# jessicabonnie/dandd

Hardware: AMD Instinct MI355X
Metric: Gbp/s sketched over k-sweep (higher is better)
Workload: dtype u64; 1 GPU; cfg2: 10 x 50 Mbp synthetic FASTA on this GPU (10 over 1 GPU(s)) resident in HBM, HLL log2m=14, k-sweep 4-40 (K=37), leaf sketches + root union + all cardinalities + delta; genomes_per_gpu=10, bases_per_genome=50000000, kmin=4, kmax=40, log2m=14, parallelism=genomes sharded over 1 GPU(s)

## Files before the change

dandd_amd/csrc/dd_api.hip:

```cpp
#include "dd_ctx.h"

thread_local std::string g_err;

extern "C" {

int dd_abi_version(void) { return DD_ABI_VERSION; }

const char* dd_last_error(void) { return g_err.c_str(); }

dd_ctx* dd_create(int device, int log2m, int canonical) {
    if (log2m < 4 || log2m > 20) {
        fail(DD_EINVAL, "log2m=%d outside 4..20", log2m);
        return nullptr;
    }
    int ndev = 0;
    hipError_t e = hipGetDeviceCount(&ndev);
    if (e != hipSuccess || ndev <= 0) {
        fail(DD_ENODEV, "no HIP device visible (%s): libdandd_hip has no CPU path",
             e == hipSuccess ? "device count 0" : hipGetErrorString(e));
        return nullptr;
    }
    if (device < 0 || device >= ndev) {
        fail(DD_ENODEV, "device %d not in 0..%d", device, ndev - 1);
        return nullptr;
// ... 6 lines not shown
    if (strncmp(prop.gcnArchName, "gfx950", 6) != 0) {
        fail(DD_ENODEV, "device %d is %s; this library is built for gfx950 only", device,
             prop.gcnArchName);
        return nullptr;
    }
    dd_ctx* c = new dd_ctx();
    c->device = device;
    c->p = log2m;
    c->canonical = canonical ? 1 : 0;
    c->bucket_budget = std::min<size_t>((size_t)48 << 30, std::max<size_t>((size_t)16 << 30, prop.totalGlobalMem / 6));
    DeviceGuard g(device);
    if (hipEventCreateWithFlags(&c->stage[0].free, hipEventDisableTiming) != hipSuccess ||
        hipEventCreateWithFlags(&c->stage[1].free, hipEventDisableTiming) != hipSuccess) {
        fail(DD_ENODEV, "hipEventCreate failed");
        delete c;
        return nullptr;
    }
    return c;
}

void dd_destroy(dd_ctx* c) {
    if (!c) return;
    DeviceGuard g(c->device);
    (void)hipStreamSynchronize(c->stream);
    (void)dd_comm_destroy(c);
    for (auto& v : c->spans)
        for (auto& s : v) {
            (void)hipEventDestroy(s.a);
            (void)hipEventDestroy(s.b);
        }
    for (auto e : c->pool) (void)hipEventDestroy(e);
    for (auto& pe : c->plans) pe.jobtab.release();
    for (DevBuf* b : {&c->tokens, &c->scratch, &c->tables, &c->fasta, &c->regs, &c->ptrs, &c->hist,
                      &c->est, &c->ord, &c->bitmaps, &c->bigmaps, &c->exact, &c->buckets, &c->gram, &c->synth, &c->masks, &c->emit, &c->hits, &c->pat[0], &c->pat[1]})
        b->release();
    for (StageSet& s : c->stage) {
        if (s.free) (void)hipEventDestroy(s.free);
        for (HostBuf* b : {&s.tables, &s.jobs, &s.rows}) b->release();
    }
    c->ingest.release();
    for (int i = 0; i < 8; ++i)
        if (c->side[i]) {
            (void)hipStreamDestroy(c->side[i]);
            (void)hipEventDestroy(c->side_done[i]);
        }
    if (c->side_go) (void)hipEventDestroy(c->side_go);
    delete c;
}

int dd_set_stream(dd_ctx* c, void* hip_stream) {
    if (check_ctx(c)) return DD_EINVAL;
    hipStream_t next = static_cast<hipStream_t>(hip_stream);
    if (next != c->stream) {
        DeviceGuard g(c->device);
        DD_HIP(hipDeviceSynchronize());
        c->stream = next;
    }
    return DD_OK;
}

int dd_synchronize(dd_ctx* c) {
    if (check_ctx(c)) return DD_EINVAL;
    DeviceGuard g(c->device);
    DD_HIP(hipStreamSynchronize(c->stream));
    return DD_OK;
}

// ... 109 lines not shown
```

dandd_amd/csrc/dd_ctx.h:

```cpp
#pragma once
#include "../../include/dandd_hip.h"
#include <sched.h>
#include <stdarg.h>
#include <stdio.h>
#include <stdlib.h>
#include <string.h>
#include <algorithm>
#include <string>
#include <thread>
#include <vector>
#include "dd_common.h"
#include "dd_io.h"
#include "dd_kernels.h"
#include "dd_plan.h"

extern thread_local std::string g_err;
inline int fail(int code, const char* fmt, ...) {
    char buf[512];
    va_list ap;
    va_start(ap, fmt), vsnprintf(buf, sizeof buf, fmt, ap), va_end(ap);
    g_err = buf;
    return code;
}
#define DD_HIP(expr)                                                                                                     \
// ... 42 lines not shown
    std::vector<dd::FileBuf*> file_pool;
    hipStream_t copy_stream_b = nullptr;
    hipStream_t copy_stream = nullptr, out_stream = nullptr;
    PipeSet pipe[2];
    bool no_gpu_inflate = false;
    int inflate_refusals = 0;
    bool inflate_retry = false;
    bool inflate_retry_counts = false;
    struct TextSink { uint8_t* const* out; const size_t* caps; size_t* lens; bool short_buffer; };
    TextSink* text_sink = nullptr;
    int calls = 0;
    double ms[4] = {0, 0, 0, 0};
    void release() {
        for (dd::FileBuf*& fb : file_pool) delete fb, fb = nullptr;
        for (PipeSet& s : pipe) s.release();
        for (hipStream_t* s : {&copy_stream, &copy_stream_b, &out_stream})
            if (*s) (void)hipStreamDestroy(*s), *s = nullptr;
    }
};

struct StageSet { HostBuf tables, jobs, rows; hipEvent_t free = nullptr; };

struct dd_ctx {
    int device = 0, p = 14, canonical = 1;
    hipStream_t stream = nullptr;
    bool timing = false;
    std::vector<TimedSpan> spans[DD_KERNEL_COUNT];
    std::vector<hipEvent_t> pool;
    DevBuf tokens, scratch, tables, fasta, regs, ptrs, hist, est, ord, bitmaps, bigmaps, exact, buckets, gram, synth;
    DevBuf masks;
    DevBuf emit;
    DevBuf hits;
    DevBuf pat[2];
    StageSet stage[2];
    int stage_cur = 0;
    struct PlanEntry {
        bool valid = false;
        int kmin = 0, kmax = 0;
        std::vector<size_t> sizes;
        dd::PlanKnobs knobs;
        std::vector<dd::SweepClass> classes;
        std::vector<size_t> job_off;
        DevBuf jobtab;
        unsigned long long last_use = 0;
    };
    PlanEntry plans[8];
    unsigned long long plan_clock = 0;
    IngestState ingest;
    hipStream_t side[8] = {};
    hipEvent_t side_done[8] = {}, side_go = nullptr;
    size_t bucket_budget = (size_t)16 << 30;
    uint64_t st_tokens = 0, st_updates = 0;
    int st_blocks = 0;
    int k2_path = 0;
    void* comm = nullptr;
    int comm_rank = 0, comm_world = 1;
    unsigned long long comm_calls[2] = {0, 0};
};
struct DeviceGuard {
    int prev = -1;
    explicit DeviceGuard(int dev) {
        (void)hipGetDevice(&prev);
        if (prev != dev) (void)hipSetDevice(dev);
        else prev = -1;
    }
    ~DeviceGuard() { if (prev >= 0) (void)hipSetDevice(prev); }
// ... 149 lines not shown
```

dandd_amd/csrc/dd_kernels.h:

```cpp
#pragma once
#include <atomic>
#include <type_traits>
#include <vector>
#include <hip/hip_runtime.h>
#include <stddef.h>
#include <stdint.h>

namespace dd {

template <typename F>
void dispatch_bool(bool b, const F& f) {
    if (b) f(std::true_type{});
    else f(std::false_type{});
}
template <auto Kern, int STATIC_LDS = 0, typename... Args>
void launch_full_lds(dim3 grid, dim3 block, size_t lds_bytes, hipStream_t st, Args... args) {
    static std::atomic<unsigned long long> allowed{0};
    int dev = 0;
    (void)hipGetDevice(&dev);
    const unsigned long long bit = 1ull << (dev & 63);
    if (!(allowed.load(std::memory_order_relaxed) & bit)) {
        if (hipFuncSetAttribute(reinterpret_cast<const void*>(Kern), hipFuncAttributeMaxDynamicSharedMemorySize, 160 * 1024 - STATIC_LDS) != hipSuccess)
            (void)hipGetLastError();
        allowed.fetch_or(bit, std::memory_order_relaxed);
// ... 3 lines not shown

struct TokenStream {
    uint32_t* codes;
    uint32_t* bad;
    unsigned long long* ntok;
};

constexpr int kPackThreads = 256;
constexpr int kPackBytesPerThread = 64;
constexpr int kPackChunk = kPackThreads * kPackBytesPerThread;
constexpr int kSegTokens = 64;

inline size_t pack_chunks(size_t n) { return (n + kPackChunk - 1) / kPackChunk; }
inline size_t pack_scratch_bytes(size_t n) { return ((pack_chunks(n) + 1) * 4 + 2) * sizeof(long long); }
inline size_t codes_words(size_t n) { return ((n + 63) / 64 + 1) * 4; }
inline size_t bad_words(size_t n) { return ((n + 63) / 64 + 1) * 2; }

struct PackGenome {
    const uint8_t* fa;
    size_t n;
    size_t nchunks;
    long long* scratch;
    TokenStream out;
};
void launch_pack_batch(const PackGenome* tab_dev, int ngenomes, size_t max_chunks, hipStream_t st);

struct SweepGenome {
    const uint32_t* codes;
    const uint32_t* bad;
    const unsigned long long* ntok;
    uint8_t* regs;
    uint32_t* bitmap;
    uint32_t* bigmap;
};

constexpr int kBitmapMaxK = 9;
constexpr int kBitmapWords = 10924;
constexpr int kBitmapStride = 11008;
inline constexpr int bitmap_offset(int k) {
    int off = 0;
    for (int j = 1; j < k; ++j) off += (j < 3) ? 1 : (1 << (2 * j - 5));
    return off;
}
inline constexpr int bitmap_words(int k) { return (k < 3) ? 1 : (1 << (2 * k - 5)); }
constexpr int kBigmapMinK = 10, kBigmapMaxK = 11;
constexpr int kBigmapSliceWords = 1 << 15;
inline constexpr int bigmap_last_k(int log2m) { return log2m >= 20 ? 11 : (log2m >= 19 ? 10 : 0); }
inline constexpr int bigmap_bits(int k, bool canon) { return (canon && (k & 1)) ? 2 * k - 1 : 2 * k; }
inline constexpr int bigmap_slices(int k, bool canon) { return 1 << (bigmap_bits(k, canon) - 20); }
inline constexpr size_t bigmap_offset_words(int k, bool canon) {
    size_t off = 0;
    for (int j = kBigmapMinK; j < k; ++j) off += (size_t)bigmap_slices(j, canon) * kBigmapSliceWords;
    return off;
}
struct SweepJob {
    int genome;
    int kfirst;
    int nk;
    int krow;
    unsigned tile_begin, tile_end;
    int slice;
};
constexpr int kBucketMode = 5;
constexpr int kBucketFromLog2m = 17;
constexpr unsigned kRaiseQueueRecords = 128;
constexpr unsigned kRaiseQueueBytes = 16 * kRaiseQueueRecords * 4;
struct SweepPlan {
    int log2m;
    int canonical;
    int threads;
    int lds_bytes;
    int queue_off = 0;
    int mode;
    int logg = 0;
    int nb_log2 = 0;
    unsigned cap_chunks = 0;
    int nepochs = 0;
};
void launch_sweep(const SweepGenome* genomes_dev, const SweepJob* jobs_dev, int njobs, int kclass,
                  const SweepPlan& plan, hipStream_t st);

struct BucketRow {
    uint8_t* regs;
    uint32_t* area;
    uint32_t* cursor;
    uint32_t* fill;
    uint16_t* seg;
    uint8_t* filter;
    uint32_t* ones;
};
struct ScatterParams {
    const BucketRow* rows;
    int K;
    int logg;
    unsigned cap_chunks;
    int nb_log2;
};
void launch_scatter(const SweepGenome* genomes_dev, const SweepJob* jobs_dev, int njobs, int kclass,
                    const SweepPlan& plan, const ScatterParams& sp, hipStream_t st, bool first_epoch);
void launch_replay(const BucketRow* rows_dev, int ngenomes, int K, int k0, int nks, const SweepPlan& plan, hipStream_t st, bool first_epoch);
int sweep_max_lds_bytes();
void launch_bitmap(const SweepGenome* genomes_dev, const SweepJob* jobs_dev, int njobs, int kfirst, int klast,
                   int canonical, hipStream_t st);
void launch_bigmap(const SweepGenome* genomes_dev, const SweepJob* jobs_dev, int njobs, int canonical, hipStream_t st);
void launch_bigmap_finish(const SweepGenome* genomes_dev, int ngenomes, int kfirst, int klast, int kmin, int log2m,
                          int canonical, hipStream_t st);
void launch_bitmap_finish(const SweepGenome* genomes_dev, int ngenomes, int kfirst, int klast, int kmin,
                          int log2m, hipStream_t st);

void launch_union(const uint8_t* const* in_dev, int n, size_t len, uint8_t* out_dev, hipStream_t st);
void launch_hist(const uint8_t* regs_dev, int njobs, int log2m, uint32_t* hist_dev, hipStream_t st);
void launch_progressive(const uint8_t* leaf_dev, int n, int K, int log2m, const int32_t* ord_dev,
                        int norder, uint32_t* hist_dev, hipStream_t st);
// ... 201 lines not shown
```

dandd_amd/csrc/dd_plan.h:

```cpp
#pragma once
#include <stddef.h>

#include <vector>

#include "dd_kernels.h"

namespace dd {

constexpr int kBitmapClass = -1;
constexpr int kBigmapClass = -2;

struct SweepClass {
    int kclass;
    int kfirst, klast;
    SweepPlan plan;
    std::vector<SweepJob> jobs;
    std::vector<size_t> epoch_begin;
};

struct PlanKnobs {
    size_t bucket_e0_tiles = 0;
    size_t bucket_emax_tiles = 0;
    size_t bucket_cap_chunks = 0;
    size_t bucket_budget = (size_t)16 << 30;
    bool bigmap_any_size = false;
    static PlanKnobs from_env();
    bool operator==(const PlanKnobs& o) const {
        return bucket_e0_tiles == o.bucket_e0_tiles && bucket_emax_tiles == o.bucket_emax_tiles && bucket_cap_chunks == o.bucket_cap_chunks &&
               bucket_budget == o.bucket_budget && bigmap_any_size == o.bigmap_any_size;
    }
};

bool plan_bigmap_range(int log2m, int kmin, int kmax, const PlanKnobs& knobs, const size_t* nbytes, int ngenomes, int* ka, int* kb);
std::vector<SweepClass> plan_sweep(int log2m, int canonical, const size_t* nbytes, int ngenomes, int kmin,
                                   int kmax, const PlanKnobs& knobs);

struct BucketLayout {
    int K = 0, per_genome = 0;
    std::vector<int> slot;
    size_t table = 0, cursors = 0, filters = 0, ones = 0, fills = 0, areas = 0;
    size_t cursor_stride = 256, filter_bytes = 0, ones_bytes = 0, fill_bytes = 0, seg_off = 0, area_bytes = 0;
    size_t zero_begin = 0, zero_bytes = 0, total = 0;
};
BucketLayout bucket_layout(const std::vector<SweepClass>& classes, int log2m, int ngenomes, int kmin, int kmax);
void bucket_rows(const BucketLayout& lay, char* base, uint8_t* regs, int log2m, int ngenomes, BucketRow* rows);

}
```

dandd_amd/csrc/dd_plan.hip:

```cpp
#include "dd_plan.h"

#include <stdlib.h>

#include <algorithm>

namespace dd {

PlanKnobs PlanKnobs::from_env() {
    PlanKnobs k;
    k.bigmap_any_size = getenv("DD_BIGMAP_ANY_SIZE") != nullptr;
    if (const char* e = getenv("DD_BUCKET_E0")) k.bucket_e0_tiles = (size_t)std::max(1, atoi(e));
    if (const char* e = getenv("DD_BUCKET_EMAX")) k.bucket_emax_tiles = (size_t)std::max(1, atoi(e));
    if (const char* e = getenv("DD_BUCKET_CAP")) k.bucket_cap_chunks = (size_t)std::max(1, atoi(e));
    if (const char* e = getenv("DD_BUCKET_GB")) k.bucket_budget = (size_t)std::max(1, atoi(e)) << 30;
    return k;
}

namespace {

constexpr int kThreads = 1024;
constexpr size_t kTileTokens = (size_t)kThreads * kSegTokens;

size_t tiles_of(size_t nbytes) { return (nbytes + kTileTokens - 1) / kTileTokens; }
size_t align_to(size_t v, size_t a) { return (v + a - 1) / a * a; }

SweepJob make_job(int genome, int kfirst, int nk, int kmin, size_t t0, size_t t1) {
    SweepJob j;
    j.genome = genome;
    j.kfirst = kfirst;
    j.nk = nk;
    j.krow = kfirst - kmin;
    j.tile_begin = (unsigned)t0;
    j.tile_end = (unsigned)t1;
    j.slice = 0;
    return j;
}

}

bool plan_bigmap_range(int log2m, int kmin, int kmax, const PlanKnobs& knobs, const size_t* nbytes, int ngenomes, int* ka, int* kb) {
    int last = log2m >= kBucketFromLog2m ? bigmap_last_k(log2m) : 0;
    size_t total = 0;
    for (int g = 0; g < ngenomes; ++g) total += nbytes[g];
    const size_t avg = ngenomes > 0 ? total / (size_t)ngenomes : 0;
    const size_t tiles = (size_t)1 << std::max(0, log2m - 17);
    while (!knobs.bigmap_any_size && last >= kBigmapMinK && avg < tiles * ((size_t)1 << (2 * last))) --last;
    const int a = std::max(kmin, kBigmapMinK), b = std::min(kmax, last);
    if (a > b) return false;
    if (ka) *ka = a;
    if (kb) *kb = b;
    return true;
}

std::vector<SweepClass> plan_sweep(int log2m, int canonical, const size_t* nbytes, int ngenomes, int kmin,
                                   int kmax, const PlanKnobs& knobs) {
    std::vector<SweepClass> classes;
    if (ngenomes <= 0 || kmin < 1 || kmax > 64 || kmin > kmax) return classes;
    const int p = log2m;
    const size_t m = (size_t)1 << p;
    const bool bucket_mode = p >= kBucketFromLog2m;
    const size_t lds_budget = std::max<size_t>(80 * 1024, m);
    const int slots = (int)std::min<size_t>(64, lds_budget / m);
    const bool use_bitmaps = kmin <= kBitmapMaxK;
    int big_ka = 0, big_kb = 0;
    const bool use_big = plan_bigmap_range(p, kmin, kmax, knobs, nbytes, ngenomes, &big_ka, &big_kb);

    const int lo0 = use_big ? big_kb + 1 : (use_bitmaps ? kBitmapMaxK + 1 : 1);
    const struct { int kc, ka, kb; } class_tab[6] = {
        {kBitmapClass, 1, use_bitmaps ? kBitmapMaxK : 0}, {kBigmapClass, big_ka, use_big ? big_kb : 0},
        {0, lo0, 16}, {1, 17, 32}, {3, 33, 48}, {2, 49, 64}};

    size_t total_tiles = 0, max_tiles = 0;
    for (int g = 0; g < ngenomes; ++g) {
        total_tiles += tiles_of(nbytes[g]);
        max_tiles = std::max(max_tiles, tiles_of(nbytes[g]));
    }

    int bucket_logg = std::max(1, p - 17);
    while (bucket_logg > 0 && (m >> bucket_logg) / 2 < 16) --bucket_logg;
    const int nb_log2 = std::max(0, p - 16);
    std::vector<size_t> epoch_edge;
    size_t epoch_longest = 0, bucket_row_tokens = 0;
    if (bucket_mode) {
        int bucketed_ks = 0;
// ... 201 lines not shown
```

dandd_amd/csrc/dd_sketch_api.hip:

```cpp
#include "dd_ctx.h"

static int ensure_side_streams(dd_ctx* c, int n) {
    if (!c->side_go) DD_HIP(hipEventCreateWithFlags(&c->side_go, hipEventDisableTiming));
    for (int i = 0; i < std::min(n, 8); ++i) {
        if (c->side[i]) continue;
        DD_HIP(hipStreamCreateWithFlags(&c->side[i], hipStreamNonBlocking));
        DD_HIP(hipEventCreateWithFlags(&c->side_done[i], hipEventDisableTiming));
    }
    return DD_OK;
}

struct SideLanes {
    dd_ctx* c;
    int lane = 0;
    template <class F>
    int run(bool fork, F&& launch) {
        const int l = lane & 7;
        if (!fork) return launch(c->stream), DD_OK;
        DD_HIP(hipStreamWaitEvent(c->side[l], c->side_go, 0));
        launch(c->side[l]);
        DD_HIP(hipEventRecord(c->side_done[l], c->side[l]));
        DD_HIP(hipStreamWaitEvent(c->stream, c->side_done[l], 0));
        ++lane;
        return DD_OK;
    }
};

struct Bitmaps { uint32_t* small = nullptr; uint32_t* big = nullptr; size_t big_stride = 0; };
static int reserve_bitmaps(dd_ctx* c, const dd::PlanKnobs& knobs, const size_t* nbytes, int ngenomes, int kmin, int kmax, Bitmaps& bm) {
    int rc, ka = 0, kb = 0;
    if (kmin <= dd::kBitmapMaxK) {
        const size_t bbytes = (size_t)ngenomes * dd::kBitmapStride * sizeof(uint32_t);
        if ((rc = c->bitmaps.reserve(bbytes))) return rc;
        bm.small = static_cast<uint32_t*>(c->bitmaps.p);
        DD_HIP(hipMemsetAsync(bm.small, 0, bbytes, c->stream));
    }
    if (dd::plan_bigmap_range(c->p, kmin, kmax, knobs, nbytes, ngenomes, &ka, &kb)) {
        bm.big_stride = dd::bigmap_offset_words(kb + 1, c->canonical != 0);
        const size_t bbytes = (size_t)ngenomes * bm.big_stride * sizeof(uint32_t);
        if ((rc = c->bigmaps.reserve(bbytes))) return rc;
        bm.big = static_cast<uint32_t*>(c->bigmaps.p);
        DD_HIP(hipMemsetAsync(bm.big, 0, bbytes, c->stream));
    }
    return DD_OK;
}

static int cached_plan(dd_ctx* c, StageSet& stage, const dd::PlanKnobs& knobs, const size_t* nbytes, int ngenomes, int kmin, int kmax, dd_ctx::PlanEntry** out) {
    dd_ctx::PlanEntry* pc = &c->plans[0];
    for (auto& pe : c->plans) {
        if (pe.valid && pe.kmin == kmin && pe.kmax == kmax && pe.knobs == knobs && pe.sizes.size() == (size_t)ngenomes &&
            std::equal(pe.sizes.begin(), pe.sizes.end(), nbytes)) {
            pe.last_use = ++c->plan_clock;
            *out = &pe;
            return DD_OK;
        }
        if (pe.last_use < pc->last_use) pc = &pe;
    }
    pc->last_use = ++c->plan_clock;
    pc->valid = false;
    pc->classes = dd::plan_sweep(c->p, c->canonical, nbytes, ngenomes, kmin, kmax, knobs);
    size_t job_bytes = 0;
    pc->job_off.assign(pc->classes.size(), 0);
    for (size_t i = 0; i < pc->classes.size(); ++i) {
        pc->job_off[i] = job_bytes;
        job_bytes += align_up(sizeof(dd::SweepJob) * pc->classes[i].jobs.size(), 256);
    }
    int rc;
    if ((rc = pc->jobtab.reserve(job_bytes))) return rc;
    if ((rc = stage.jobs.reserve(job_bytes))) return rc;
    for (size_t i = 0; i < pc->classes.size(); ++i)
        if ((rc = upload(c, stage.jobs, static_cast<char*>(pc->jobtab.p) + pc->job_off[i], pc->classes[i].jobs.data(),
                         sizeof(dd::SweepJob) * pc->classes[i].jobs.size(), pc->job_off[i])))
            return rc;
    pc->kmin = kmin;
    pc->kmax = kmax;
    pc->knobs = knobs;
    pc->sizes.assign(nbytes, nbytes + ngenomes);
    pc->valid = true;
    *out = pc;
    return DD_OK;
}

static int upload_bucket_rows(dd_ctx* c, StageSet& stage, const std::vector<dd::SweepClass>& classes, int ngenomes, int kmin, int kmax, uint8_t* regs_dev,
                              const dd::BucketRow** rows_dev) {
    const dd::BucketLayout lay = dd::bucket_layout(classes, c->p, ngenomes, kmin, kmax);
    if (!lay.total) return DD_OK;
    std::vector<dd::BucketRow> rtab((size_t)ngenomes * lay.K);
    int rc;
    if ((rc = c->buckets.reserve(lay.total))) return rc;
    if ((rc = stage.rows.reserve(lay.cursors - lay.table))) return rc;
    char* bb = static_cast<char*>(c->buckets.p);
    dd::bucket_rows(lay, bb, regs_dev, c->p, ngenomes, rtab.data());
    DD_HIP(hipMemsetAsync(bb + lay.zero_begin, 0, lay.zero_bytes, c->stream));
    if ((rc = upload(c, stage.rows, bb + lay.table, rtab.data(), sizeof(dd::BucketRow) * rtab.size(), 0))) return rc;
    *rows_dev = reinterpret_cast<const dd::BucketRow*>(bb + lay.table);
    return DD_OK;
}

static void launch_lds_class(dd_ctx* c, const dd::SweepClass& sc, const dd::SweepGenome* gt, const dd::SweepJob* jt, int ngenomes, int kmin, hipStream_t ks) {
    if (sc.kclass == dd::kBitmapClass) {
        dd::launch_bitmap(gt, jt, (int)sc.jobs.size(), sc.kfirst, sc.klast, c->canonical, ks);
        dd::launch_bitmap_finish(gt, ngenomes, sc.kfirst, sc.klast, kmin, c->p, ks);
    } else if (sc.kclass == dd::kBigmapClass) {
        dd::launch_bigmap(gt, jt, (int)sc.jobs.size(), c->canonical, ks);
        dd::launch_bigmap_finish(gt, ngenomes, sc.kfirst, sc.klast, kmin, c->p, c->canonical, ks);
    } else {
        dd::launch_sweep(gt, jt, (int)sc.jobs.size(), sc.kclass, sc.plan, ks);
    }
}

static int launch_classes(dd_ctx* c, const dd_ctx::PlanEntry& plan, const dd::SweepGenome* gtab, const dd::BucketRow* rows, int ngenomes, int kmin, int kmax, int* blocks) {
    const int K = kmax - kmin + 1;
    size_t lds_jobs = 0;
    int lds_classes = 0, nepochs = 0, rc;
    for (const dd::SweepClass& sc : plan.classes) {
        if (sc.plan.mode != dd::kBucketMode) lds_jobs += sc.jobs.size(), ++lds_classes;
        else nepochs = sc.plan.nepochs;
    }
    const bool side = lds_classes > 1 && lds_jobs < 12000, side_b = nepochs > 1;
    if ((side || side_b) && (rc = ensure_side_streams(c, side_b ? (int)plan.classes.size() : lds_classes))) return rc;
    Span phase(c, DD_KERNEL_SWEEP, side || side_b);
    if (side || side_b) DD_HIP(hipEventRecord(c->side_go, c->stream));
    SideLanes lanes{c};
    for (size_t i = 0; i < plan.classes.size(); ++i) {
        const dd::SweepClass& sc = plan.classes[i];
        const dd::SweepJob* jobs = reinterpret_cast<const dd::SweepJob*>(static_cast<char*>(plan.jobtab.p) + plan.job_off[i]);
        const bool bucket = sc.plan.mode == dd::kBucketMode, on_lane = side_b || (side && !bucket);
        rc = lanes.run(on_lane, [&](hipStream_t ks) {
            if (!bucket) {
                Span span(c, DD_KERNEL_SWEEP, !on_lane);
                launch_lds_class(c, sc, gtab, jobs, ngenomes, kmin, ks);
            }
            const dd::ScatterParams sp{rows, K, sc.plan.logg, sc.plan.cap_chunks, sc.plan.nb_log2};
            for (int e = 0; bucket && e < sc.plan.nepochs; ++e) {
                const size_t j0 = sc.epoch_begin[e], j1 = sc.epoch_begin[e + 1];
                if (j1 == j0) continue;
                Span span(c, DD_KERNEL_SWEEP, !on_lane);
                dd::launch_scatter(gtab, jobs + j0, (int)(j1 - j0), sc.kclass, sc.plan, sp, ks, e == 0);
                dd::launch_replay(rows, ngenomes, K, sc.kfirst - kmin, sc.klast - sc.kfirst + 1, sc.plan, ks, e == 0);
            }
        });
        if (rc) return rc;
        *blocks += (int)sc.jobs.size();
    }
    DD_HIP(hipGetLastError());
    return DD_OK;
}

extern "C" {

int dd_sketch_device(dd_ctx* c, const uint8_t* const* fasta_dev, const size_t* nbytes, int ngenomes,
                     int kmin, int kmax, uint8_t* regs_dev) {
    if (check_ctx(c)) return DD_EINVAL;
    if (ngenomes < 0 || !regs_dev || (ngenomes && (!fasta_dev || !nbytes)))
        return fail(DD_EINVAL, "null argument");
    if (kmin < 1 || kmax > 64 || kmin > kmax) return fail(DD_EINVAL, "k range %d..%d outside 1..64", kmin, kmax);
    uint64_t tokens_ub = 0;
    for (int g = 0; g < ngenomes; ++g) {
        if (nbytes[g] && !fasta_dev[g]) return fail(DD_EINVAL, "genome %d: null buffer", g);
        if (reinterpret_cast<uintptr_t>(fasta_dev[g]) & 15)
            return fail(DD_EINVAL, "genome %d: device buffer must be 16-byte aligned", g);
        tokens_ub += nbytes[g];
    }
    DeviceGuard guard(c->device);
    const size_t K = (size_t)(kmax - kmin + 1), m = (size_t)1 << c->p;
    DD_HIP(hipMemsetAsync(regs_dev, 0, (size_t)ngenomes * K * m, c->stream));
    if (!ngenomes) return DD_OK;

    dd::PlanKnobs knobs = dd::PlanKnobs::from_env();
    if (!getenv("DD_BUCKET_GB")) knobs.bucket_budget = c->bucket_budget;
    std::vector<dd::PackGenome> ptab;
    size_t max_chunks = 0;
    Bitmaps bm;
    int rc;
    if ((rc = layout_tokens(c, fasta_dev, nbytes, ngenomes, ptab, max_chunks))) return rc;
    if ((rc = reserve_bitmaps(c, knobs, nbytes, ngenomes, kmin, kmax, bm))) return rc;
    std::vector<dd::SweepGenome> gtab(ngenomes);
    for (int g = 0; g < ngenomes; ++g) {
        const dd::TokenStream& ts = ptab[g].out;
        gtab[g] = dd::SweepGenome{ts.codes, ts.bad, ts.ntok, regs_dev + (size_t)g * K * m,
                                  bm.small ? bm.small + (size_t)g * dd::kBitmapStride : nullptr,
                                  bm.big ? bm.big + (size_t)g * bm.big_stride : nullptr};
    }

    const size_t pack_off = align_up(sizeof(dd::SweepGenome) * ngenomes, 256);
    const size_t gtab_bytes = pack_off + align_up(sizeof(dd::PackGenome) * ngenomes, 256);
    if ((rc = c->tables.reserve(gtab_bytes))) return rc;
    StageSet& stage = c->stage[c->stage_cur ^= 1];
    DD_HIP(hipEventSynchronize(stage.free));
    if ((rc = stage.tables.reserve(gtab_bytes))) return rc;
    char* tdev = static_cast<char*>(c->tables.p);
    if ((rc = upload(c, stage.tables, tdev, gtab.data(), sizeof(dd::SweepGenome) * ngenomes, 0))) return rc;
    if ((rc = upload(c, stage.tables, tdev + pack_off, ptab.data(), sizeof(dd::PackGenome) * ngenomes, pack_off))) return rc;
    {
        Span sp(c, DD_KERNEL_PACK);
        dd::launch_pack_batch(reinterpret_cast<const dd::PackGenome*>(tdev + pack_off), ngenomes, max_chunks, c->stream);
    }
    DD_HIP(hipGetLastError());

    dd_ctx::PlanEntry* plan = nullptr;
    const dd::BucketRow* rows_dev = nullptr;
    int blocks = 0;
    if ((rc = cached_plan(c, stage, knobs, nbytes, ngenomes, kmin, kmax, &plan))) return rc;
    if ((rc = upload_bucket_rows(c, stage, plan->classes, ngenomes, kmin, kmax, regs_dev, &rows_dev))) return rc;
    DD_HIP(hipEventRecord(stage.free, c->stream));
    if ((rc = launch_classes(c, *plan, reinterpret_cast<const dd::SweepGenome*>(tdev), rows_dev, ngenomes, kmin, kmax, &blocks))) return rc;
    c->st_tokens = tokens_ub;
    c->st_updates = tokens_ub * (uint64_t)K;
    c->st_blocks = blocks;
    return DD_OK;
}

int dd_sketch_buffer(dd_ctx* c, const uint8_t* fasta, size_t nbytes, int kmin, int kmax, uint8_t* regs) {
    if (check_ctx(c)) return DD_EINVAL;
    if (!regs || (nbytes && !fasta)) return fail(DD_EINVAL, "null argument");
    if (kmin < 1 || kmax > 64 || kmin > kmax) return fail(DD_EINVAL, "k range %d..%d outside 1..64", kmin, kmax);
    DeviceGuard guard(c->device);
    const size_t K = (size_t)(kmax - kmin + 1), m = (size_t)1 << c->p;
    int rc;
    dd::FileBuf fq;
    if (dd::has_plus_line(fasta, nbytes)) {
        if (!fq.reserve(nbytes + 16)) return fail(DD_ENOMEM, "out of host memory");
        fq.len = nbytes = dd::fastq_to_fasta(fasta, nbytes, fq.p);
        fasta = fq.p;
    }
    if ((rc = c->fasta.reserve(nbytes + 16))) return rc;
    if ((rc = c->regs.reserve(K * m))) return rc;
    if (nbytes) DD_HIP(hipMemcpyAsync(c->fasta.p, fasta, nbytes, hipMemcpyHostToDevice, c->stream));
    const uint8_t* ptrs[1] = {static_cast<const uint8_t*>(c->fasta.p)};
    const size_t ns[1] = {nbytes};
    if ((rc = dd_sketch_device(c, ptrs, ns, 1, kmin, kmax, static_cast<uint8_t*>(c->regs.p)))) return rc;
    DD_HIP(hipMemcpyAsync(regs, c->regs.p, K * m, hipMemcpyDeviceToHost, c->stream));
    DD_HIP(hipStreamSynchronize(c->stream));
    return DD_OK;
}

}
```

dandd_amd/csrc/dd_sweep.hip:

```cpp
#include "dd_common.h"
#include "dd_kernels.h"
#include "dd_k1.h"

namespace dd {
namespace {

template <int KC, bool CANON, bool CHECK, typename Win>
DD_D void sweep_token(const Win& win, int run, int kfirst, int nk, int p, RaiseQueue& s) {
    constexpr bool QUEUE = KC != 0;
    asm volatile("" : "+s"(nk));
    int j = 0;
#pragma unroll 1
    for (; j + 1 < nk; j += 2) {
        const int k = kfirst + j;
        const bool ok0 = !CHECK || run >= k, ok1 = !CHECK || run > k;
        const unsigned long long okm0 = CHECK ? __builtin_amdgcn_ballot_w64(run >= k) : ~0ull, okm1 = CHECK ? __builtin_amdgcn_ballot_w64(run > k) : ~0ull;
        if (CHECK && !okm0) return;
        sweep_update2<QUEUE, CHECK>(s, (uint32_t)j, win.template hash<CANON>(k), okm0, ok0,
                                    (uint32_t)j + 1u, win.template hash<CANON>(k + 1), okm1, ok1, p);
    }
    if (j < nk) {
        const int k = kfirst + j;
        const unsigned long long okm = CHECK ? __builtin_amdgcn_ballot_w64(run >= k) : ~0ull;
        if (!CHECK || okm) sweep_update<QUEUE, CHECK>(s, (uint32_t)j, win.template hash<CANON>(k), okm, !CHECK || run >= k, p);
    }
}

template <int KC, bool CANON>
__global__ __launch_bounds__(1024) void sweep_kernel(const SweepGenome* __restrict__ genomes,
                                                    const SweepJob* __restrict__ jobs, int p, uint32_t queue_off) {
    lds_starts_at_zero();
    const SweepJob job = jobs[blockIdx.x];
    const SweepGenome g = genomes[job.genome];
    const int nk = job.nk, kfirst = job.kfirst;
    const uint32_t m = 1u << p;
    const unsigned long long ntok = gload8u(g.ntok);
    uint8_t* const slab = g.regs + ((size_t)job.krow << p);

    TileIn next;
    fetch_tile(g, job, ntok, job.tile_begin, next);

    {
        uint4* z = reinterpret_cast<uint4*>(g_lds);
        const uint32_t n16 = (uint32_t)nk * (m >> 4);
        for (uint32_t i = threadIdx.x; i < n16; i += blockDim.x) z[i] = load16_fresh(slab + (size_t)i * 16);
    }
    __syncthreads();

    const int kmaxg = kfirst + nk - 1;
    RaiseQueue s;
    s.base = queue_off + (uint32_t)__builtin_amdgcn_readfirstlane(threadIdx.x >> 6) * (kRaiseQueueRecords * 4u);
    s.dense = (KC != 0 && queue_off) ? kRaiseDense : 0u;
    s.waiting = 0;

    for (unsigned tile = job.tile_begin; tile < job.tile_end; ++tile) {
        const TileIn cur = next;
        fetch_tile(g, job, ntok, tile + 1, next);
        if (!__any(cur.live)) continue;
        SweepWindows<KC> win;
        walk_segment(cur, win, [&](auto clean, int run) {
            if constexpr (decltype(clean)::value) {
                sweep_token<KC, CANON, false>(win, 0, kfirst, nk, p, s);
            } else {
                if (__all(run >= kmaxg)) sweep_token<KC, CANON, false>(win, run, kfirst, nk, p, s);
                else sweep_token<KC, CANON, true>(win, run, kfirst, nk, p, s);
            }
        });
    }
    if (s.dense) sweep_drain(s);
    __syncthreads();

    const uint4* l4 = reinterpret_cast<const uint4*>(g_lds);
    uint32_t* gw = reinterpret_cast<uint32_t*>(slab);
    const uint32_t n16 = (uint32_t)nk * (m >> 4);
    for (uint32_t i = threadIdx.x; i < n16; i += blockDim.x) {
        const uint4 lv = l4[i];
        const uint4 gv = load16_fresh(slab + (size_t)i * 16);
        const uint32_t l[4] = {lv.x, lv.y, lv.z, lv.w};
        const uint32_t o[4] = {gv.x, gv.y, gv.z, gv.w};
#pragma unroll
        for (int q = 0; q < 4; ++q) {
            uint32_t old = o[q];
            uint32_t mx = bmax4(old, l[q]);
            while (mx != old) {
                uint32_t prev = gcas32(&gw[4 * i + q], old, mx);
                if (prev == old) break;
                old = prev;
                mx = bmax4(old, l[q]);
            }
        }
    }
}

__constant__ int c_bitmap_off[kBitmapMaxK + 2] = {0, bitmap_offset(1), bitmap_offset(2), bitmap_offset(3),
                                                 bitmap_offset(4), bitmap_offset(5), bitmap_offset(6),
                                                 bitmap_offset(7), bitmap_offset(8), bitmap_offset(9),
                                                 kBitmapWords};
static_assert(kBitmapMaxK == 9 && bitmap_offset(9) + bitmap_words(9) == kBitmapWords &&
              kBitmapWords + kBitmapMaxK < kBitmapStride, "bitmap layout");

template <bool CANON>
__global__ __launch_bounds__(1024) __attribute__((amdgpu_num_sgpr(72))) void bitmap_kernel(const SweepGenome* __restrict__ genomes,
                                                     const SweepJob* __restrict__ jobs) {
    const SweepJob job = jobs[blockIdx.x];
    const SweepGenome g = genomes[job.genome];
    const int kfirst = job.kfirst, klast = job.kfirst + job.nk - 1;
    const unsigned long long ntok = gload8u(g.ntok);
    const int w0 = c_bitmap_off[kfirst], w1 = c_bitmap_off[klast + 1];
    uint32_t* const bits = reinterpret_cast<uint32_t*>(g_lds) - w0;
    uint32_t kmask = __builtin_amdgcn_readfirstlane(((2u << klast) - 1u) & ~((1u << kfirst) - 1u));
    uint32_t* const complete = g.bitmap + kBitmapWords;
    __shared__ uint32_t have[kBitmapMaxK + 2];
    __shared__ uint32_t flagged;
    if (threadIdx.x == 0) {
        uint32_t f = 0;
        for (int k = kfirst; k <= klast; ++k)
            if (load4_fresh(complete + k)) f |= 1u << k;
        flagged = f;
    }
    if (threadIdx.x <= kBitmapMaxK) have[threadIdx.x] = 0;
    __syncthreads();
    kmask = __builtin_amdgcn_readfirstlane(kmask & ~flagged);
// ... 156 lines not shown
#pragma unroll
        for (int w = 0; w < 4; ++w) {
            const uint32_t bw = ((w & 2) ? sb.y : sb.x) >> ((w & 1) * 16);
#pragma unroll 4
            for (int i = 0; i < 16; ++i) {
                const uint32_t c = (cws[w] >> (2 * i)) & 3u;
                run = ((bw >> i) & 1u) ? 0 : run + 1;
                win.push(c);
                record(bigmap_index<CANON>(win.fw, win.rc, k), run >= k);
            }
        }
    }
    __syncthreads();
    for (int i = threadIdx.x; i < kBigmapSliceWords; i += blockDim.x) {
        const uint32_t mine = bits[i];
        if (mine && (mine & ~load4_fresh(home + i))) gor32(home + i, mine);
    }
}

template <bool CANON>
__global__ __launch_bounds__(1024) void bigmap_finish_kernel(const SweepGenome* __restrict__ genomes,
                                                            int kfirst, int kmin, int p, int tile_log2) {
    lds_starts_at_zero();
    const SweepGenome g = genomes[blockIdx.y];
    const int k = kfirst + (int)blockIdx.x;
    const uint32_t b = blockIdx.z;
    const uint32_t* bm = g.bigmap + bigmap_offset_words(k, CANON);
    const uint32_t nw = (uint32_t)bigmap_slices(k, CANON) * kBigmapSliceWords;
    finish_tile(g.regs + ((size_t)(k - kmin) << p) + ((size_t)b << tile_log2), tile_log2, b, p, [&](const auto& emit) {
        for_each_set_bit(bm, nw, [&](uint32_t idx) { emit(bigmap_kmer<CANON>(idx, k)); });
    });
}

}

int sweep_max_lds_bytes() { return 160 * 1024; }

void launch_bitmap(const SweepGenome* genomes, const SweepJob* jobs, int njobs, int kfirst, int klast,
                   int canonical, hipStream_t st) {
    if (njobs <= 0 || kfirst < 1 || klast > kBitmapMaxK || klast < kfirst) return;
    const size_t lds = (size_t)(bitmap_offset(klast) + bitmap_words(klast) - bitmap_offset(kfirst)) * 4;
    dispatch_bool(canonical != 0, [&](auto cn) {
        launch_full_lds<bitmap_kernel<decltype(cn)::value>, 256>(dim3((unsigned)njobs), dim3(1024), lds, st, genomes, jobs);
    });
}

void launch_bitmap_finish(const SweepGenome* genomes, int ngenomes, int kfirst, int klast, int kmin, int log2m,
                          hipStream_t st) {
    if (ngenomes <= 0 || klast < kfirst) return;
    const int tile_log2 = std::min(log2m, 16);
    hipLaunchKernelGGL(bitmap_finish_kernel, dim3((unsigned)(klast - kfirst + 1), (unsigned)ngenomes, 1u << (log2m - tile_log2)), dim3(1024),
                       (size_t)1 << tile_log2, st, genomes, kfirst, kmin, log2m, tile_log2);
}

void launch_bigmap(const SweepGenome* genomes, const SweepJob* jobs, int njobs, int canonical, hipStream_t st) {
    if (njobs <= 0) return;
    dispatch_bool(canonical != 0, [&](auto cn) {
        launch_full_lds<bigmap_kernel<decltype(cn)::value>>(dim3((unsigned)njobs), dim3(1024), (size_t)kBigmapSliceWords * 4, st, genomes, jobs);
    });
}

void launch_bigmap_finish(const SweepGenome* genomes, int ngenomes, int kfirst, int klast, int kmin, int log2m,
                          int canonical, hipStream_t st) {
    if (ngenomes <= 0 || klast < kfirst) return;
    const int tile_log2 = std::min(log2m, 17);
    const dim3 grid((unsigned)(klast - kfirst + 1), (unsigned)ngenomes, 1u << (log2m - tile_log2));
    dispatch_bool(canonical != 0, [&](auto cn) {
        launch_full_lds<bigmap_finish_kernel<decltype(cn)::value>>(grid, dim3(1024), (size_t)1 << tile_log2, st, genomes, kfirst, kmin, log2m, tile_log2);
    });
}

void launch_sweep(const SweepGenome* genomes, const SweepJob* jobs, int njobs, int kclass,
                  const SweepPlan& plan, hipStream_t st) {
    if (njobs <= 0) return;
    dispatch_kc_canon(kclass, plan.canonical, [&](auto kc, auto cn) {
        launch_full_lds<sweep_kernel<decltype(kc)::value, decltype(cn)::value>>(dim3((unsigned)njobs), dim3((unsigned)plan.threads), (size_t)plan.lds_bytes, st,
                                                                                genomes, jobs, plan.log2m, (uint32_t)plan.queue_off);
    });
}

}
```

Before: 37.98 Gbp/s.

## Skip sweep work for small k once sketches saturate to the universe sketch

For k in 10..14, the HLL registers of the complete k-mer universe are computed once per context and cached. During the merge step, each sweep block compares its merged register rows against the universe rows. When a row matches exactly, a per-genome per-k saturation flag is set. Later sweep jobs read these flags and drop the leading saturated k values, returning early when nothing is left. The skip only applies when a genome is at least eight times the universe size. It adds a universe load and compare in the merge loop, extra syncs, and a one-time universe build, and blocks that run concurrently may not see the flags in time to benefit.

```diff
diff --git a/dandd_amd/csrc/dd_api.hip b/dandd_amd/csrc/dd_api.hip
--- a/dandd_amd/csrc/dd_api.hip
+++ b/dandd_amd/csrc/dd_api.hip
@@ -62,7 +62,7 @@
     for (auto e : c->pool) (void)hipEventDestroy(e);
     for (auto& pe : c->plans) pe.jobtab.release();
     for (DevBuf* b : {&c->tokens, &c->scratch, &c->tables, &c->fasta, &c->regs, &c->ptrs, &c->hist,
-                      &c->est, &c->ord, &c->bitmaps, &c->bigmaps, &c->exact, &c->buckets, &c->gram, &c->synth, &c->masks, &c->emit, &c->hits, &c->pat[0], &c->pat[1]})
+                      &c->est, &c->ord, &c->bitmaps, &c->bigmaps, &c->exact, &c->buckets, &c->gram, &c->synth, &c->masks, &c->emit, &c->hits, &c->pat[0], &c->pat[1], &c->universe})
         b->release();
     for (StageSet& s : c->stage) {
         if (s.free) (void)hipEventDestroy(s.free);
diff --git a/dandd_amd/csrc/dd_ctx.h b/dandd_amd/csrc/dd_ctx.h
--- a/dandd_amd/csrc/dd_ctx.h
+++ b/dandd_amd/csrc/dd_ctx.h
@@ -98,6 +98,8 @@
     DevBuf emit;
     DevBuf hits;
     DevBuf pat[2];
+    DevBuf universe;
+    bool universe_built[dd::kSatMaxK - dd::kSatMinK + 1] = {};
     StageSet stage[2];
     int stage_cur = 0;
     struct PlanEntry {
diff --git a/dandd_amd/csrc/dd_kernels.h b/dandd_amd/csrc/dd_kernels.h
--- a/dandd_amd/csrc/dd_kernels.h
+++ b/dandd_amd/csrc/dd_kernels.h
@@ -59,6 +59,7 @@
     uint8_t* regs;
     uint32_t* bitmap;
     uint32_t* bigmap;
+    uint32_t* sat;
 };
 
 constexpr int kBitmapMaxK = 9;
@@ -104,8 +105,13 @@
     unsigned cap_chunks = 0;
     int nepochs = 0;
 };
+constexpr int kSatMinK = 10, kSatMaxK = 14;
+inline constexpr size_t universe_size(int k, bool canon) {
+    return canon ? ((size_t)1 << (2 * k - 1)) + ((k & 1) ? 0 : ((size_t)1 << (k - 1))) : (size_t)1 << (2 * k);
+}
+void launch_universe(uint8_t* row_dev, int k, int log2m, int canonical, hipStream_t st);
 void launch_sweep(const SweepGenome* genomes_dev, const SweepJob* jobs_dev, int njobs, int kclass,
-                  const SweepPlan& plan, hipStream_t st);
+                  const SweepPlan& plan, const uint8_t* universe_dev, int universe_last_k, hipStream_t st);
 
 struct BucketRow {
     uint8_t* regs;
diff --git a/dandd_amd/csrc/dd_plan.h b/dandd_amd/csrc/dd_plan.h
--- a/dandd_amd/csrc/dd_plan.h
+++ b/dandd_amd/csrc/dd_plan.h
@@ -24,14 +24,18 @@
     size_t bucket_cap_chunks = 0;
     size_t bucket_budget = (size_t)16 << 30;
     bool bigmap_any_size = false;
+    bool saturate_any_size = false;
+    bool no_saturate = false;
     static PlanKnobs from_env();
     bool operator==(const PlanKnobs& o) const {
         return bucket_e0_tiles == o.bucket_e0_tiles && bucket_emax_tiles == o.bucket_emax_tiles && bucket_cap_chunks == o.bucket_cap_chunks &&
-               bucket_budget == o.bucket_budget && bigmap_any_size == o.bigmap_any_size;
+               bucket_budget == o.bucket_budget && bigmap_any_size == o.bigmap_any_size &&
+               saturate_any_size == o.saturate_any_size && no_saturate == o.no_saturate;
     }
 };
 
 bool plan_bigmap_range(int log2m, int kmin, int kmax, const PlanKnobs& knobs, const size_t* nbytes, int ngenomes, int* ka, int* kb);
+int plan_saturate_last_k(int log2m, int canonical, int kmin, int kmax, const PlanKnobs& knobs, const size_t* nbytes, int ngenomes);
 std::vector<SweepClass> plan_sweep(int log2m, int canonical, const size_t* nbytes, int ngenomes, int kmin,
                                    int kmax, const PlanKnobs& knobs);
 
diff --git a/dandd_amd/csrc/dd_plan.hip b/dandd_amd/csrc/dd_plan.hip
--- a/dandd_amd/csrc/dd_plan.hip
+++ b/dandd_amd/csrc/dd_plan.hip
@@ -9,6 +9,8 @@
 PlanKnobs PlanKnobs::from_env() {
     PlanKnobs k;
     k.bigmap_any_size = getenv("DD_BIGMAP_ANY_SIZE") != nullptr;
+    k.saturate_any_size = getenv("DD_SATURATE_ANY_SIZE") != nullptr;
+    k.no_saturate = getenv("DD_NO_SATURATE") != nullptr;
     if (const char* e = getenv("DD_BUCKET_E0")) k.bucket_e0_tiles = (size_t)std::max(1, atoi(e));
     if (const char* e = getenv("DD_BUCKET_EMAX")) k.bucket_emax_tiles = (size_t)std::max(1, atoi(e));
     if (const char* e = getenv("DD_BUCKET_CAP")) k.bucket_cap_chunks = (size_t)std::max(1, atoi(e));
@@ -50,6 +52,15 @@
     if (ka) *ka = a;
     if (kb) *kb = b;
     return true;
+}
+
+int plan_saturate_last_k(int log2m, int canonical, int kmin, int kmax, const PlanKnobs& knobs, const size_t* nbytes, int ngenomes) {
+    if (knobs.no_saturate || log2m < 4 || log2m >= kBucketFromLog2m || ngenomes <= 0) return 0;
+    size_t longest = 0;
+    for (int g = 0; g < ngenomes; ++g) longest = std::max(longest, nbytes[g]);
+    int last = std::min(kmax, kSatMaxK);
+    while (!knobs.saturate_any_size && last >= kSatMinK && longest < 8 * universe_size(last, canonical != 0)) --last;
+    return last >= std::max(kmin, kSatMinK) ? last : 0;
 }
 
 std::vector<SweepClass> plan_sweep(int log2m, int canonical, const size_t* nbytes, int ngenomes, int kmin,
diff --git a/dandd_amd/csrc/dd_sketch_api.hip b/dandd_amd/csrc/dd_sketch_api.hip
--- a/dandd_amd/csrc/dd_sketch_api.hip
+++ b/dandd_amd/csrc/dd_sketch_api.hip
@@ -26,14 +26,15 @@
     }
 };
 
-struct Bitmaps { uint32_t* small = nullptr; uint32_t* big = nullptr; size_t big_stride = 0; };
-static int reserve_bitmaps(dd_ctx* c, const dd::PlanKnobs& knobs, const size_t* nbytes, int ngenomes, int kmin, int kmax, Bitmaps& bm) {
+struct Bitmaps { uint32_t* small = nullptr; uint32_t* big = nullptr; size_t big_stride = 0; uint32_t* sat = nullptr; };
+static int reserve_bitmaps(dd_ctx* c, const dd::PlanKnobs& knobs, const size_t* nbytes, int ngenomes, int kmin, int kmax, size_t sat_words, Bitmaps& bm) {
     int rc, ka = 0, kb = 0;
-    if (kmin <= dd::kBitmapMaxK) {
-        const size_t bbytes = (size_t)ngenomes * dd::kBitmapStride * sizeof(uint32_t);
+    if (kmin <= dd::kBitmapMaxK || sat_words) {
+        const size_t words = kmin <= dd::kBitmapMaxK ? (size_t)ngenomes * dd::kBitmapStride : 0, bbytes = (words + sat_words) * sizeof(uint32_t);
         if ((rc = c->bitmaps.reserve(bbytes))) return rc;
-        bm.small = static_cast<uint32_t*>(c->bitmaps.p);
-        DD_HIP(hipMemsetAsync(bm.small, 0, bbytes, c->stream));
+        if (words) bm.small = static_cast<uint32_t*>(c->bitmaps.p);
+        if (sat_words) bm.sat = static_cast<uint32_t*>(c->bitmaps.p) + words;
+        DD_HIP(hipMemsetAsync(c->bitmaps.p, 0, bbytes, c->stream));
     }
     if (dd::plan_bigmap_range(c->p, kmin, kmax, knobs, nbytes, ngenomes, &ka, &kb)) {
         bm.big_stride = dd::bigmap_offset_words(kb + 1, c->canonical != 0);
@@ -97,7 +98,21 @@
     return DD_OK;
 }
 
-static void launch_lds_class(dd_ctx* c, const dd::SweepClass& sc, const dd::SweepGenome* gt, const dd::SweepJob* jt, int ngenomes, int kmin, hipStream_t ks) {
+static int ensure_universe(dd_ctx* c, int kfirst, int last_k) {
+    if (!last_k) return DD_OK;
+    const size_t m = (size_t)1 << c->p;
+    int rc;
+    if ((rc = c->universe.reserve((size_t)(dd::kSatMaxK - dd::kSatMinK + 1) * m))) return rc;
+    for (int k = std::max(kfirst, dd::kSatMinK); k <= last_k; ++k) {
+        if (c->universe_built[k - dd::kSatMinK]) continue;
+        dd::launch_universe(static_cast<uint8_t*>(c->universe.p) + (size_t)(k - dd::kSatMinK) * m, k, c->p, c->canonical, c->stream);
+        DD_HIP(hipGetLastError());
+        c->universe_built[k - dd::kSatMinK] = true;
+    }
+    return DD_OK;
+}
+
+static void launch_lds_class(dd_ctx* c, const dd::SweepClass& sc, const dd::SweepGenome* gt, const dd::SweepJob* jt, int ngenomes, int kmin, int sat_last_k, hipStream_t ks) {
     if (sc.kclass == dd::kBitmapClass) {
         dd::launch_bitmap(gt, jt, (int)sc.jobs.size(), sc.kfirst, sc.klast, c->canonical, ks);
         dd::launch_bitmap_finish(gt, ngenomes, sc.kfirst, sc.klast, kmin, c->p, ks);
@@ -105,11 +120,11 @@
         dd::launch_bigmap(gt, jt, (int)sc.jobs.size(), c->canonical, ks);
         dd::launch_bigmap_finish(gt, ngenomes, sc.kfirst, sc.klast, kmin, c->p, c->canonical, ks);
     } else {
-        dd::launch_sweep(gt, jt, (int)sc.jobs.size(), sc.kclass, sc.plan, ks);
-    }
-}
-
-static int launch_classes(dd_ctx* c, const dd_ctx::PlanEntry& plan, const dd::SweepGenome* gtab, const dd::BucketRow* rows, int ngenomes, int kmin, int kmax, int* blocks) {
+        dd::launch_sweep(gt, jt, (int)sc.jobs.size(), sc.kclass, sc.plan, static_cast<const uint8_t*>(c->universe.p), sat_last_k, ks);
+    }
+}
+
+static int launch_classes(dd_ctx* c, const dd_ctx::PlanEntry& plan, const dd::SweepGenome* gtab, const dd::BucketRow* rows, int ngenomes, int kmin, int kmax, int sat_last_k, int* blocks) {
     const int K = kmax - kmin + 1;
     size_t lds_jobs = 0;
     int lds_classes = 0, nepochs = 0, rc;
@@ -129,7 +144,7 @@
         rc = lanes.run(on_lane, [&](hipStream_t ks) {
             if (!bucket) {
                 Span span(c, DD_KERNEL_SWEEP, !on_lane);
-                launch_lds_class(c, sc, gtab, jobs, ngenomes, kmin, ks);
+                launch_lds_class(c, sc, gtab, jobs, ngenomes, kmin, sat_last_k, ks);
             }
             const dd::ScatterParams sp{rows, K, sc.plan.logg, sc.plan.cap_chunks, sc.plan.nb_log2};
             for (int e = 0; bucket && e < sc.plan.nepochs; ++e) {
@@ -174,13 +189,16 @@
     Bitmaps bm;
     int rc;
     if ((rc = layout_tokens(c, fasta_dev, nbytes, ngenomes, ptab, max_chunks))) return rc;
-    if ((rc = reserve_bitmaps(c, knobs, nbytes, ngenomes, kmin, kmax, bm))) return rc;
+    const int sat_last_k = dd::plan_saturate_last_k(c->p, c->canonical, kmin, kmax, knobs, nbytes, ngenomes);
+    if ((rc = reserve_bitmaps(c, knobs, nbytes, ngenomes, kmin, kmax, sat_last_k ? (size_t)ngenomes * K : 0, bm))) return rc;
+    if ((rc = ensure_universe(c, kmin, sat_last_k))) return rc;
     std::vector<dd::SweepGenome> gtab(ngenomes);
     for (int g = 0; g < ngenomes; ++g) {
         const dd::TokenStream& ts = ptab[g].out;
         gtab[g] = dd::SweepGenome{ts.codes, ts.bad, ts.ntok, regs_dev + (size_t)g * K * m,
                                   bm.small ? bm.small + (size_t)g * dd::kBitmapStride : nullptr,
-                                  bm.big ? bm.big + (size_t)g * bm.big_stride : nullptr};
+                                  bm.big ? bm.big + (size_t)g * bm.big_stride : nullptr,
+                                  bm.sat ? bm.sat + (size_t)g * K : nullptr};
     }
 
     const size_t pack_off = align_up(sizeof(dd::SweepGenome) * ngenomes, 256);
@@ -204,7 +222,7 @@
     if ((rc = cached_plan(c, stage, knobs, nbytes, ngenomes, kmin, kmax, &plan))) return rc;
     if ((rc = upload_bucket_rows(c, stage, plan->classes, ngenomes, kmin, kmax, regs_dev, &rows_dev))) return rc;
     DD_HIP(hipEventRecord(stage.free, c->stream));
-    if ((rc = launch_classes(c, *plan, reinterpret_cast<const dd::SweepGenome*>(tdev), rows_dev, ngenomes, kmin, kmax, &blocks))) return rc;
+    if ((rc = launch_classes(c, *plan, reinterpret_cast<const dd::SweepGenome*>(tdev), rows_dev, ngenomes, kmin, kmax, sat_last_k, &blocks))) return rc;
     c->st_tokens = tokens_ub;
     c->st_updates = tokens_ub * (uint64_t)K;
     c->st_blocks = blocks;
diff --git a/dandd_amd/csrc/dd_sweep.hip b/dandd_amd/csrc/dd_sweep.hip
--- a/dandd_amd/csrc/dd_sweep.hip
+++ b/dandd_amd/csrc/dd_sweep.hip
@@ -28,14 +28,33 @@
 
 template <int KC, bool CANON>
 __global__ __launch_bounds__(1024) void sweep_kernel(const SweepGenome* __restrict__ genomes,
-                                                    const SweepJob* __restrict__ jobs, int p, uint32_t queue_off) {
+                                                    const SweepJob* __restrict__ jobs, int p, uint32_t queue_off,
+                                                    const uint8_t* __restrict__ universe, int universe_last_k) {
     lds_starts_at_zero();
     const SweepJob job = jobs[blockIdx.x];
     const SweepGenome g = genomes[job.genome];
-    const int nk = job.nk, kfirst = job.kfirst;
+    int nk = job.nk, kfirst = job.kfirst, krow = job.krow;
     const uint32_t m = 1u << p;
+
+    int nsat = 0;
+    if constexpr (KC == 0) {
+        if (g.sat && kfirst <= universe_last_k) nsat = min(nk, universe_last_k - kfirst + 1);
+        if (nsat) {
+            uint32_t* const word = reinterpret_cast<uint32_t*>(g_lds);
+            if (threadIdx.x == 0) {
+                uint32_t d = 0;
+                while (d < (uint32_t)nsat && load4_fresh(g.sat + krow + d)) ++d;
+                *word = d;
+            }
+            __syncthreads();
+            const int d = __builtin_amdgcn_readfirstlane((int)*word);
+            __syncthreads();
+            kfirst += d, nk -= d, krow += d, nsat -= d;
+            if (nk == 0) return;
+        }
+    }
     const unsigned long long ntok = gload8u(g.ntok);
-    uint8_t* const slab = g.regs + ((size_t)job.krow << p);
+    uint8_t* const slab = g.regs + ((size_t)krow << p);
 
     TileIn next;
     fetch_tile(g, job, ntok, job.tile_begin, next);
@@ -73,11 +92,19 @@
     const uint4* l4 = reinterpret_cast<const uint4*>(g_lds);
     uint32_t* gw = reinterpret_cast<uint32_t*>(slab);
     const uint32_t n16 = (uint32_t)nk * (m >> 4);
+    const uint32_t nsat16 = (uint32_t)nsat * (m >> 4);
+    const uint8_t* const urow = universe + ((size_t)(kfirst - kSatMinK) << p);
+    uint32_t short_rows = 0;
     for (uint32_t i = threadIdx.x; i < n16; i += blockDim.x) {
         const uint4 lv = l4[i];
         const uint4 gv = load16_fresh(slab + (size_t)i * 16);
         const uint32_t l[4] = {lv.x, lv.y, lv.z, lv.w};
         const uint32_t o[4] = {gv.x, gv.y, gv.z, gv.w};
+        uint32_t u[4] = {0u, 0u, 0u, 0u}, below = 0;
+        if (KC == 0 && i < nsat16) {
+            const uint4 uv = gload16(urow + (size_t)i * 16);
+            u[0] = uv.x, u[1] = uv.y, u[2] = uv.z, u[3] = uv.w;
+        }
 #pragma unroll
         for (int q = 0; q < 4; ++q) {
             uint32_t old = o[q];
@@ -88,6 +115,19 @@
                 old = prev;
                 mx = bmax4(old, l[q]);
             }
+            below |= mx ^ u[q];
+        }
+        if (KC == 0 && i < nsat16 && below) short_rows |= 1u << (i >> (p - 4));
+    }
+    if constexpr (KC == 0) {
+        if (nsat) {
+            uint32_t* const word = reinterpret_cast<uint32_t*>(g_lds);
+            __syncthreads();
+            if (threadIdx.x == 0) *word = 0u;
+            __syncthreads();
+            if (short_rows) atomicOr(word, short_rows);
+            __syncthreads();
+            if (threadIdx.x < (uint32_t)nsat && !((*word >> threadIdx.x) & 1u)) gor32(g.sat + krow + threadIdx.x, 1u);
         }
     }
 }
@@ -310,6 +350,55 @@
     });
 }
 
+template <bool CANON>
+__global__ __launch_bounds__(1024) void universe_kernel(uint8_t* __restrict__ row, int k, int p) {
+    lds_starts_at_zero();
+    const uint32_t m = 1u << p;
+    uint4* z = reinterpret_cast<uint4*>(g_lds);
+    for (uint32_t i = threadIdx.x; i < (m >> 4); i += blockDim.x) z[i] = make_uint4(0, 0, 0, 0);
+    __syncthreads();
+    const uint32_t n = 1u << (2 * k);
+    for (uint32_t x = blockIdx.x * blockDim.x + threadIdx.x; x < n; x += gridDim.x * blockDim.x) {
+        if (CANON) {
+            uint32_t r = __brev(x);
+            r = ((r >> 1) & 0x55555555u) | ((r & 0x55555555u) << 1);
+            r = (~r) >> (32 - 2 * k);
+            if (r < x) continue;
+        }
+        const Probe q = probe(wang64_fast<true>(x), p);
+        lds_raise(q.hi >> (32 - p), rho_of(q, p));
+    }
+    __syncthreads();
+    const uint4* l4 = reinterpret_cast<const uint4*>(g_lds);
+    uint32_t* gw = reinterpret_cast<uint32_t*>(row);
+    for (uint32_t i = threadIdx.x; i < (m >> 4); i += blockDim.x) {
+        const uint4 lv = l4[i];
+        const uint4 gv = load16_fresh(row + (size_t)i * 16);
+        const uint32_t l[4] = {lv.x, lv.y, lv.z, lv.w};
+        const uint32_t o[4] = {gv.x, gv.y, gv.z, gv.w};
+#pragma unroll
+        for (int q = 0; q < 4; ++q) {
+            uint32_t old = o[q];
+            uint32_t mx = bmax4(old, l[q]);
+            while (mx != old) {
+                uint32_t prev = gcas32(&gw[4 * i + q], old, mx);
+                if (prev == old) break;
+                old = prev;
+                mx = bmax4(old, l[q]);
+            }
+        }
+    }
+}
+
+}
+
+void launch_universe(uint8_t* row_dev, int k, int log2m, int canonical, hipStream_t st) {
+    if (k < kSatMinK || k > kSatMaxK || log2m < 4 || log2m > 16) return;
+    (void)hipMemsetAsync(row_dev, 0, (size_t)1 << log2m, st);
+    const unsigned grid = std::min(1024u, 1u << (2 * k - 16));
+    dispatch_bool(canonical != 0, [&](auto cn) {
+        hipLaunchKernelGGL(universe_kernel<decltype(cn)::value>, dim3(grid), dim3(1024), (size_t)1 << log2m, st, row_dev, k, log2m);
+    });
 }
 
 int sweep_max_lds_bytes() { return 160 * 1024; }
@@ -349,12 +438,13 @@
 }
 
 void launch_sweep(const SweepGenome* genomes, const SweepJob* jobs, int njobs, int kclass,
-                  const SweepPlan& plan, hipStream_t st) {
+                  const SweepPlan& plan, const uint8_t* universe, int universe_last_k, hipStream_t st) {
     if (njobs <= 0) return;
+    if (!universe || kclass != 0) universe_last_k = 0;
     dispatch_kc_canon(kclass, plan.canonical, [&](auto kc, auto cn) {
         launch_full_lds<sweep_kernel<decltype(kc)::value, decltype(cn)::value>>(dim3((unsigned)njobs), dim3((unsigned)plan.threads), (size_t)plan.lds_bytes, st,
-                                                                                genomes, jobs, plan.log2m, (uint32_t)plan.queue_off);
-    });
-}
-
-}
+                                                                                genomes, jobs, plan.log2m, (uint32_t)plan.queue_off, universe, universe_last_k);
+    });
+}
+
+}
```

New measurement: 38.93 Gbp/s, median of 6. 1.03x the previous value.
